# Vigilans/GomokuAI

Measured on AMD Instinct MI355X. Metric: board-evals/s, higher is better.
Workload: dtype int32; 1 GPU; batched AC-automaton position eval (K1), 65536 random-opening boards per GPU, 15x15, inputs resident in HBM; boards_per_gpu=65536, parallelism=boards sharded by rank, no collective, launch=hipGraph replay of the K steps

## Files before the change

### gomokuai_amd/csrc/capi.hip

```cpp
#include <algorithm>
#include <mutex>
#include <cstring>
#include <string>
#include <vector>

#include "capi_common.h"

namespace gmk {

static thread_local char g_error[512] = "";

void set_error(const char* fmt, ...) {
    va_list ap;
    va_start(ap, fmt);
    vsnprintf(g_error, sizeof g_error, fmt, ap);
    va_end(ap);
}

DeviceState& device_state() {
    static DeviceState s;
    return s;
}

}

using gmk::device_state;
using gmk::production_automaton;

extern "C" const char* gmk_last_error(void) { return gmk::g_error; }

namespace gmk {
namespace {
struct PoolBlock { void* p; size_t bytes; bool used; unsigned long long freed_at; };
unsigned long long g_pool_clock = 0;
std::mutex g_pool_mutex;
std::vector<PoolBlock> g_pool;
constexpr size_t kPoolMinBytes = size_t(16) << 20, kPoolCapBytes = size_t(224) << 30;
bool g_pool_poison = false;
size_t pool_idle_cap(size_t idle) {
    size_t free_bytes = 0, total = 0;
    if (hipMemGetInfo(&free_bytes, &total) != hipSuccess) { (void)hipGetLastError(); return kPoolCapBytes; }
    return std::min(kPoolCapBytes, (free_bytes + idle) / 4 * 3);
}
size_t pool_idle_bytes() { size_t t = 0; for (const PoolBlock& b : g_pool) if (!b.used) t += b.bytes; return t; }
void pool_drop_idle(size_t keep) {
    while (pool_idle_bytes() > keep) {
        size_t at = g_pool.size();
        for (size_t i = 0; i < g_pool.size(); ++i) if (!g_pool[i].used && (at == g_pool.size() || g_pool[i].freed_at < g_pool[at].freed_at)) at = i;
        if (at == g_pool.size()) return;
        (void)hipFree(g_pool[at].p);
        g_pool.erase(g_pool.begin() + static_cast<long>(at));
    }
}
}
// ... 90 lines not shown
    gmk::device_pool_release();
    (void)hipFree(st.d_trans);
    (void)hipFree(st.d_records);
    st = gmk::DeviceState{};
    return GMK_OK;
}

extern "C" int gmk_device_info(int* cu_count, size_t* hbm_bytes, char* name, int name_cap) {
    gmk::DeviceState& st = device_state();
    if (!st.ready) { gmk::set_error("gmk_init has not succeeded"); return GMK_ERR_STATE; }
    hipDeviceProp_t prop;
    GMK_HIP_CHECK(hipGetDeviceProperties(&prop, st.device));
    if (cu_count) *cu_count = prop.multiProcessorCount;
    if (hbm_bytes) *hbm_bytes = prop.totalGlobalMem;
    if (name && name_cap > 0) {
        std::strncpy(name, prop.name[0] ? prop.name : prop.gcnArchName, static_cast<size_t>(name_cap) - 1);
        name[name_cap - 1] = 0;
    }
    return GMK_OK;
}

extern "C" int gmk_tables_info(gmk_table_info* info) {
    if (!info) return GMK_ERR_ARG;
    const gmk::PatternAutomaton& a = production_automaton();
    const gmk::DeviceTables& t = a.device();
    info->n_patterns = t.n_patterns;
    info->n_states = t.n_states;
    info->dat_size = static_cast<int32_t>(a.base().size());
    info->max_emissions = t.max_emissions;
    info->trans_words = static_cast<int32_t>(t.trans.size());
    info->emit_words = static_cast<int32_t>(t.emit_lists.size());
    for (int i = 0; i < 5; ++i) info->invariants[i] = a.invariants()[i];
    return GMK_OK;
}

extern "C" int gmk_tables_pattern(int i, char str[8], int* favour, int* type, int* score) {
    const auto& pats = production_automaton().patterns();
    if (i < 0 || i >= static_cast<int>(pats.size())) return GMK_ERR_ARG;
    if (str) { std::memset(str, 0, 8); std::memcpy(str, pats[i].rich.data(), pats[i].rich.size()); }
    if (favour) *favour = pats[i].favour;
    if (type) *type = pats[i].type;
    if (score) *score = pats[i].score;
    return GMK_OK;
}

extern "C" int gmk_tables_copy(uint32_t* trans, uint16_t* emit_lists, uint32_t* pattern_info) {
    const gmk::DeviceTables& t = production_automaton().device();
    if (trans) std::memcpy(trans, t.trans.data(), t.trans.size() * sizeof(uint32_t));
    if (emit_lists) std::memcpy(emit_lists, t.emit_lists.data(), t.emit_lists.size() * sizeof(uint16_t));
    if (pattern_info) std::memcpy(pattern_info, t.pattern_info.data(), t.pattern_info.size() * sizeof(uint32_t));
    return GMK_OK;
}

extern "C" int gmk_tables_copy_dat(int32_t* base, int32_t* check, int32_t* fail) {
    const gmk::PatternAutomaton& a = production_automaton();
    const size_t bytes = a.base().size() * sizeof(int32_t);
    if (base) std::memcpy(base, a.base().data(), bytes);
    if (check) std::memcpy(check, a.check().data(), bytes);
    if (fail) std::memcpy(fail, a.fail().data(), bytes);
    return GMK_OK;
}

extern "C" int gmk_tables_scan(const uint8_t* codes, int n, int32_t* patterns, int32_t* offsets, int cap) {
    if (!codes || n < 0) return GMK_ERR_ARG;
    for (int i = 0; i < n; ++i) if (codes[i] < 1 || codes[i] > 4) return GMK_ERR_ARG;
    const auto stream = production_automaton().scan(codes, n);
    int m = 0;
    for (const auto& pr : stream) {
        if (m < cap) { if (patterns) patterns[m] = pr.first; if (offsets) offsets[m] = pr.second; }
        ++m;
    }
    return m;
}
```

### gomokuai_amd/csrc/eval_kernel.hip

```cpp
#include <algorithm>
#include <cstdlib>
#include <vector>

#include "capi_common.h"

namespace {

constexpr int kBoardsPerBlock = 16;
constexpr int kGroupBoards = 16;
constexpr int kThreads = 64 * kBoardsPerBlock;
constexpr int kCells = 225;
constexpr int kQueueCap = 448;
constexpr int kMaxBlocksPerCu = 1;
constexpr int kBurstEvery = 12;
static_assert(kBurstEvery >= 1 && kBurstEvery <= kGroupBoards, "every burst of a run needs a board of the run to go with");
[[maybe_unused]] constexpr int kTimelineSlots = 8;

constexpr int kScoreWords = 4 * kCells;
constexpr int kCntWords = 3 * kCells + 1;
constexpr int kZeroWords = kScoreWords + kCntWords;
constexpr int kLineWords = 96;
constexpr int kColBase = 20, kDiagBase = 36, kAntiBase = 65;
#ifndef GMK_K1_TOTALS_COPIES
#define GMK_K1_TOTALS_COPIES 8
#endif
constexpr int kTotalsCopies = GMK_K1_TOTALS_COPIES;
constexpr int kMiscWords = 48;
constexpr int kBoardWords = kZeroWords + kLineWords + kQueueCap + kMiscWords;
static_assert(kZeroWords % 4 == 0 && kBoardWords % 4 == 0, "16-byte alignment of the per-board blocks");
constexpr int kStaticTableWords = 128 + kLineWords + 512 + 1560 + 4;

constexpr int kLaneRecordVecs = 2;
constexpr int kScanSteps = 19;

__device__ __forceinline__ int dir_stride(int dir) { return (0x0E100F01u >> (8 * dir)) & 0xFFu; }

__device__ __forceinline__ uint64_t line_symbols(uint32_t line_word, int len) {
    return 2ull | (static_cast<uint64_t>(line_word) << 2) | (0xAull << (2 * len + 2));
}

__device__ __forceinline__ const __attribute__((address_space(3))) uint32_t* lds_word(uint32_t byte_address) {
    return reinterpret_cast<const __attribute__((address_space(3))) uint32_t*>(static_cast<uintptr_t>(byte_address));
}

__device__ __forceinline__ __attribute__((address_space(3))) uint32_t* lds_word_rw(uint32_t byte_address) {
    return reinterpret_cast<__attribute__((address_space(3))) uint32_t*>(static_cast<uintptr_t>(byte_address));
}

__device__ __forceinline__ uint32_t dfa_address(uint32_t table_word, uint32_t four) {
    uint32_t addr;
    asm("v_bfi_b32 %0, %1, %2, %3" : "=v"(addr) : "s"(0x3FF3u), "v"(table_word), "v"(four));
    return addr;
}

__device__ __forceinline__ uint32_t mul24(uint32_t a, uint32_t b) {
    uint32_t r;
    asm("v_mul_u32_u24 %0, %1, %2" : "=v"(r) : "v"(a), "s"(b));
    return r;
}

__device__ __forceinline__ void store_saddr(uint32_t byte_offset, int32_t value, unsigned long long base) {
    asm volatile("global_store_dword %0, %1, %2" : : "v"(byte_offset), "v"(value), "s"(base) : "memory");
}

template <int kImm, bool kNt>
__device__ __forceinline__ void store_saddr_imm(uint32_t byte_offset, int32_t value, unsigned long long base) {
    static_assert(kImm >= 0 && kImm < 4096, "the immediate offset of a global store has 13 bits, signed");
    if (kNt) asm volatile("global_store_dword %0, %1, %2 offset:%3 nt" : : "v"(byte_offset), "v"(value), "s"(base), "n"(kImm) : "memory");
    else asm volatile("global_store_dword %0, %1, %2 offset:%3" : : "v"(byte_offset), "v"(value), "s"(base), "n"(kImm) : "memory");
}

__device__ __forceinline__ void wave_phase_fence() {
    __builtin_amdgcn_fence(__ATOMIC_RELEASE, "wavefront");
    __builtin_amdgcn_wave_barrier();
    __builtin_amdgcn_fence(__ATOMIC_ACQUIRE, "wavefront");
}

__device__ __forceinline__ void deposit_match(uint32_t w0, uint32_t w1, int cell_at, int dir, int back_step,
                                              uint32_t* s_scores, uint32_t* s_cnt, uint32_t* s_misc, uint32_t* totals ) {
    const int type = w0 & 15, fav = (w0 >> 4) & 1;
    if (type == 8) { atomicOr(&s_misc[1], fav ? 1u : 2u); return; }
    atomicAdd(&totals[type], fav ? 0x10000u : 1u);
    const int endcell = cell_at + static_cast<int>((w0 >> 27) & 1u) * back_step;
    const uint32_t score = dir >= 2 ? (w1 >> 16) : (w1 & 0xFFFFu);
    unsigned long long* pair = reinterpret_cast<unsigned long long*>(s_scores) + fav;
    const uint32_t lo_opp = fav ? score : 0u, hi_opp = fav ? 0u : score;
    const uint32_t tslot = 5u - static_cast<uint32_t>(type);
    const bool feeds = tslot < 3u;
    uint32_t* cnt = s_cnt + (feeds ? tslot : 0u) * kCells;
    const uint32_t one = 1u << (4 * (fav * 4 + dir));
    const int n_dep = (w0 >> 8) & 7;
#pragma unroll
    for (int d = 0; d < 4; ++d) {
        if (d >= n_dep) break;
        const uint32_t f = (w0 >> (11 + 4 * d)) & 15u;
        const int c = endcell + static_cast<int>(f & 7u) * back_step;
        const bool both = (f & 8u) != 0u;
        atomicAdd(&pair[2 * c], (static_cast<unsigned long long>(both ? score : hi_opp) << 32) | (both ? score : lo_opp));
        if (both && feeds) atomicAdd(&cnt[c], one);
    }
}

__device__ __forceinline__ int counter_match(uint32_t w0, int k, int want) {
    const int type = w0 & 15, len = (w0 >> 5) & 7;
    const int back = k - static_cast<int>((w0 >> 27) & 1u) - 6;
    if (!w0 || type != want || back < 0 || back >= len) return -1;
    const int n_dep = (w0 >> 8) & 7;
    bool on_q = false;
#pragma unroll
    for (int d = 0; d < 4; ++d) {
        const uint32_t f = (w0 >> (11 + 4 * d)) & 15u;
        on_q |= d < n_dep && f == (8u | static_cast<uint32_t>(back));
    }
    return on_q ? back : -1;
}

__device__ __forceinline__ void add_counter_cells(uint32_t w0, int back, int q, int stride, uint32_t* opp) {
    const int n_dep = (w0 >> 8) & 7, endcell = q + back * stride;
#pragma unroll
    for (int d = 0; d < 4; ++d) {
        const uint32_t f = (w0 >> (11 + 4 * d)) & 15u;
        if (d < n_dep && static_cast<int>(f & 7u) != back) atomicAdd(&opp[4 * (endcell - static_cast<int>(f & 7u) * stride)], 600u);
    }
}

[[maybe_unused]] constexpr int kDensTiles = 7;
__host__ __device__ constexpr int dens_kt_lo(int m) { return (((32 * m) / 15 - 3) < 0 ? 0 : (32 * m) / 15 - 3) / 2; }
__host__ __device__ constexpr int dens_kt_hi(int m) { return (((32 * m + 31) / 15 + 3) > 14 ? 14 : (32 * m + 31) / 15 + 3) / 2; }
constexpr int kWtabDy = 13, kWtabEntryWords = 4, kWtabKindWords = kWtabDy * 15 * kWtabEntryWords, kWtabWords = 2 * kWtabKindWords;
__host__ __device__ constexpr int block_weight(int dy, int dx) {
    constexpr int w[4][7] = {{1, 3, 4, 0, 4, 3, 1}, {0, 3, 5, 4, 5, 3, 0}, {0, 4, 3, 3, 3, 4, 0}, {2, 0, 0, 1, 0, 0, 2}};
    return w[dy < 0 ? -dy : dy][dx + 3];
}

typedef int v4i __attribute__((ext_vector_type(4)));
typedef int v16i __attribute__((ext_vector_type(16)));

template <bool kFull, int KIND, int M>
__device__ __forceinline__ void density_tile_pass(const uint32_t (&own_rows)[8], int n_live, int lane,
                                                  const v4i* __restrict__ s_wtab, const uint4* __restrict__ s_occ, int32_t* __restrict__ group_out,
                                                  unsigned long long& board_base , const uint2* __restrict__ s_lut, int plane_stride) {
    constexpr int lo = dens_kt_lo(M), hi = dens_kt_hi(M), nk = hi - lo + 1;
    const int n = lane & 31, h = lane >> 5;
    const uint4 occ_lo = s_occ[4 * M + 2 * h], occ_hi = s_occ[4 * M + 2 * h + 1];
    const uint32_t occ[8] = {occ_lo.x, occ_lo.y, occ_lo.z, occ_lo.w, occ_hi.x, occ_hi.y, occ_hi.z, occ_hi.w};
    const int cell = 32 * M + n, yo = (cell * 0x8889) >> 19, xo = cell - 15 * yo;
    const v4i* w = s_wtab + KIND * (kWtabKindWords / kWtabEntryWords) + (2 * lo + h - yo + 6) * 15 + xo;
    v16i acc = {0, 0, 0, 0, 0, 0, 0, 0, 0, 0, 0, 0, 0, 0, 0, 0};
#pragma unroll
    for (int k = 0; k < nk; ++k) {
        const uint32_t r = (own_rows[lo + k] >> (16 * h)) & 0x7FFFu;
        const uint2 b0 = s_lut[r & 255u], b1 = s_lut[r >> 8];
// ... 595 lines not shown
        for (int k = 0; k < 2; ++k) {
            const uint32_t job = jobs[lane * 2 + k], dir = (job >> 5) & 3u, first = (job >> 12) & 255u;
            consts[lane][2 + k] = dir == 2u ? 2u * (first % 15u) : dir == 3u ? 2u * (first / 15u) : 0u;
        }
    }
    for (int i = 0; i < 128; ++i) jobs_out[i] = jobs[i];
    for (int i = 0; i < kLineWords; ++i) pads_out[i] = ~init[i] & 0xAAAAAAAAu;
    for (int lane = 0; lane < 64; ++lane) {
        uint32_t* r = records_out + 8 * lane;
        r[0] = jobs[lane * 2]; r[1] = jobs[lane * 2 + 1];
        r[2] = init[lane]; r[3] = init[std::min(64 + lane, kLineWords - 1)];
        for (int k = 0; k < 4; ++k) r[4 + k] = consts[lane][k];
    }
    if (steps != kScanSteps) { gmk::set_error("lane jobs: %d scan steps, the kernel is built for %d", steps, kScanSteps); return GMK_ERR_STATE; }
    return GMK_OK;
}

int density_weights(int8_t* t ) {
    for (int kind = 0; kind < 2; ++kind)
        for (int dy = -3; dy <= 3; ++dy)
            for (int xo = 0; xo < 15; ++xo)
                for (int j = 0; j < 15; ++j) {
                    if (std::abs(j - xo) > 3) continue;
                    const int w = block_weight(dy, j - xo);
                    t[((static_cast<size_t>(kind) * kWtabDy + dy + 6) * 15 + xo) * 16 + j] = static_cast<int8_t>(kind == 0 ? (w != 0) : w);
                }
    for (int cell = 0; cell < 224; ++cell)
        for (int kt = dens_kt_lo(cell / 32); kt <= dens_kt_hi(cell / 32); ++kt)
            for (int h = 0; h < 2; ++h) {
                const int dy = 2 * kt + h - cell / 15;
                if (dy < -6 || dy > 6) { gmk::set_error("density weight table: dy %d of cell %d out of range", dy, cell); return GMK_ERR_STATE; }
            }
    for (int cell = 0; cell < 224; ++cell)
        for (int dy = -3; dy <= 3; ++dy) {
            const int y = cell / 15 + dy, m = cell / 32;
            if (y < 0 || y > 14) continue;
            if (y / 2 < dens_kt_lo(m) || y / 2 > dens_kt_hi(m)) { gmk::set_error("density weight table: row %d of cell %d is not covered", y, cell); return GMK_ERR_STATE; }
        }
    return GMK_OK;
}

int build_stage_image(const gmk::DeviceState& st, uint4** d_out, int* stage_vecs) {
    const size_t trans_words = static_cast<size_t>(st.n_states) * 4, record_words = static_cast<size_t>(st.n_records) * 4;
    std::vector<uint32_t> rest(kStaticTableWords + 64 * 4 * kLaneRecordVecs, 0u);
    uint32_t* jobs = rest.data(), *pads = jobs + 128, *lut = pads + kLineWords, *wtab = lut + 512, *handout = wtab + kWtabWords, *records = handout + 4;
    int rc = lane_tables(jobs, pads, records);
    if (rc != GMK_OK) return rc;
    for (uint32_t b = 0; b < 256; ++b) { lut[2 * b] = ((b & 15u) * 0x204081u) & 0x01010101u; lut[2 * b + 1] = ((b >> 4) * 0x204081u) & 0x01010101u; }
    rc = density_weights(reinterpret_cast<int8_t*>(wtab));
    if (rc != GMK_OK) return rc;
    handout[0] = 2u * kBoardsPerBlock;
    const size_t staged_words = trans_words + record_words + kStaticTableWords;
    if (staged_words % 4 != 0) { gmk::set_error("K1 tables: %zu staged words are not whole 16-byte pieces", staged_words); return GMK_ERR_STATE; }
    uint32_t* d = nullptr;
    GMK_HIP_CHECK(hipMalloc(&d, (trans_words + record_words + rest.size()) * sizeof(uint32_t)));
    GMK_HIP_CHECK(hipMemcpy(d, st.d_trans, trans_words * sizeof(uint32_t), hipMemcpyDeviceToDevice));
    GMK_HIP_CHECK(hipMemcpy(d + trans_words, st.d_records, record_words * sizeof(uint32_t), hipMemcpyDeviceToDevice));
    GMK_HIP_CHECK(hipMemcpy(d + trans_words + record_words, rest.data(), rest.size() * sizeof(uint32_t), hipMemcpyHostToDevice));
    *d_out = reinterpret_cast<uint4*>(d);
    *stage_vecs = static_cast<int>(staged_words / 4);
    return GMK_OK;
}

struct Launch { int grid, n_groups, groups_each, groups_extra; size_t lds; };

Launch plan_launch(int n, const gmk::DeviceState& st) {
    Launch l;
    l.n_groups = (n + kGroupBoards - 1) / kGroupBoards;
    l.grid = std::max(1, std::min(l.n_groups, st.cu_count * kMaxBlocksPerCu));
    l.groups_each = l.n_groups / l.grid;
    l.groups_extra = l.n_groups % l.grid;
    l.lds = static_cast<size_t>(kBoardsPerBlock * kBoardWords + st.n_states * 4 + st.n_records * 4 + kStaticTableWords) * 4;
    return l;
}

bool g_jobs_uploaded = false;
uint4* g_stage = nullptr;
int g_stage_vecs = 0;
}

extern "C" int gmk_eval_batch(const uint16_t* d_planes, int n, int32_t* d_scores, int32_t* d_density,
                              uint32_t* d_totals, int32_t* d_status, void* stream) {
    gmk::DeviceState& st = gmk::device_state();
    if (!st.ready) { gmk::set_error("gmk_init has not succeeded (no CPU fallback)"); return GMK_ERR_STATE; }
    if (n < 0 || (n > 0 && !d_planes)) { gmk::set_error("gmk_eval_batch: bad arguments"); return GMK_ERR_ARG; }
    if (n == 0) return GMK_OK;
    if (!g_jobs_uploaded) {
        const int rc = build_stage_image(st, &g_stage, &g_stage_vecs);
        if (rc != GMK_OK) return rc;
        GMK_HIP_CHECK(hipFuncSetAttribute(reinterpret_cast<const void*>(eval_positions_kernel), hipFuncAttributeMaxDynamicSharedMemorySize, 160 * 1024));
        g_jobs_uploaded = true;
    }
    const Launch l = plan_launch(n, st);
    if (l.lds > 160u * 1024u) { gmk::set_error("gmk_eval_batch: tables do not fit in LDS (%zu bytes)", l.lds); return GMK_ERR_CAPACITY; }
    static const int phase_mask = gmk::profile_env("GMK_EVAL_PHASE_MASK") ? std::atoi(gmk::profile_env("GMK_EVAL_PHASE_MASK")) : 0x7F;
    unsigned long long* d_prof = nullptr;
    static const bool stamps = gmk::profile_env("GMK_EVAL_PROFILE") != nullptr;
    if (stamps) {
        GMK_HIP_CHECK(hipMalloc(&d_prof, 16 * sizeof(unsigned long long)));
        GMK_HIP_CHECK(hipMemset(d_prof, 0, 16 * sizeof(unsigned long long)));
    }
    static const char* const timeline_path = gmk::profile_env("GMK_EVAL_TIMELINE");
    unsigned long long* d_timeline = nullptr;
    const size_t timeline_words = static_cast<size_t>(l.grid) * kBoardsPerBlock * kTimelineSlots;
    hipEvent_t tl_from = nullptr, tl_to = nullptr;
    if (timeline_path) {
        GMK_HIP_CHECK(hipMalloc(&d_timeline, timeline_words * sizeof(unsigned long long)));
        GMK_HIP_CHECK(hipMemset(d_timeline, 0, timeline_words * sizeof(unsigned long long)));
        GMK_HIP_CHECK(hipEventCreate(&tl_from));
        GMK_HIP_CHECK(hipEventCreate(&tl_to));
// ... 75 lines not shown
```

### gomokuai_amd/csrc/pattern_tables.cpp

```cpp
#include "pattern_tables.h"

#include <algorithm>
#include <deque>
#include <map>
#include <numeric>
#include <stdexcept>

namespace gmk {

namespace {

constexpr int kMaxLen = 7;
constexpr int kSymbols = 4;

std::vector<PatternRec> production_protos() {
    struct P { const char* s; int type; int score; };
    static const P table[] = {
        {"+xxxxx", Five, 9999},      {"-_oooo_", LiveFour, 9000},   {"-xoooo_", DeadFour, 2500},
        {"-o_ooo", DeadFour, 3000},  {"-oo_oo", DeadFour, 2600},    {"-~_ooo_~", LiveThree, 3000},
        {"-x^ooo_~", LiveThree, 2900}, {"-~o_oo~", LiveThree, 2800}, {"-~o~oo_~", DeadThree, 1400},
        {"-~oo~o_~", DeadThree, 1200}, {"-x_o~oo~", DeadThree, 1300}, {"-x_oo~o~", DeadThree, 1100},
        {"-xooo__~", DeadThree, 510}, {"-xoo_o_~", DeadThree, 520},  {"-xoo__o~", DeadThree, 520},
        {"-xo_oo_~", DeadThree, 530}, {"-xo__oo", DeadThree, 530},   {"-xooo__x", DeadThree, 500},
        {"-xoo_o_x", DeadThree, 500}, {"-xoo__ox", DeadThree, 500},  {"-xo_oo_x", DeadThree, 500},
// ... 300 lines not shown
        dev_.dev_prefix4[idx] = static_cast<uint16_t>(row);
    }

    {
        const int n = dev_.n_states;
        std::vector<std::vector<uint32_t>> frontier(1), next_frontier;
        frontier[0].resize(static_cast<size_t>(n));
        for (int i = 0; i < n; ++i) frontier[0][static_cast<size_t>(i)] = static_cast<uint32_t>(i);
        int length = 0;
        while (!frontier.empty()) {
            if (++length > 12) throw std::runtime_error("pattern automaton: does not forget its start state within 12 symbols");
            next_frontier.clear();
            std::vector<char> seen(static_cast<size_t>(n));
            for (const std::vector<uint32_t>& set : frontier)
                for (uint32_t sym = 0; sym < 4; ++sym) {
                    std::fill(seen.begin(), seen.end(), 0);
                    std::vector<uint32_t> image;
                    for (uint32_t st : set) {
                        const uint32_t to = dev_.trans[st * 4 + sym] & 1023u;
                        if (!seen[to]) { seen[to] = 1; image.push_back(to); }
                    }
                    if (image.size() > 1) next_frontier.push_back(std::move(image));
                }
            frontier.swap(next_frontier);
        }
        dev_.sync_symbols = length;
        if (length > 7) throw std::runtime_error("pattern automaton: needs more than 7 symbols to forget its start state");
    }
}

std::vector<std::pair<int, int>> PatternAutomaton::scan(const uint8_t* codes, int n) const {
    std::vector<std::pair<int, int>> out;
    uint32_t state = 0;
    for (int k = 0; k < n; ++k) {
        const uint32_t w = dev_.trans[state * 4 + (codes[k] - 1)];
        state = w & 1023u;
        const uint32_t li = w >> 10;
        if (li) {
            const int cnt = dev_.emit_lists[li];
            for (int e = 0; e < cnt; ++e) {
                const uint16_t v = dev_.emit_lists[li + 1 + e];
                out.emplace_back(v & 0x7fff, k - (v >> 15));
            }
        }
    }
    return out;
}

const PatternAutomaton& production_automaton() {
    static const PatternAutomaton a;
    return a;
}

}
```

### gomokuai_amd/csrc/pattern_tables.h

```cpp
#pragma once
#include <cstdint>
#if defined(__HIP__)
#include <hip/hip_runtime.h>
#endif
#include <string>
#include <vector>

namespace gmk {

enum PatternType : int { DeadOne, LiveOne, DeadTwo, LiveTwo, DeadThree, LiveThree, DeadFour, LiveFour, Five, NumPatternTypes };

struct PatternRec {
    std::string rich;
    int favour;
    int type;
    int score;
};

inline int symbol_code(char ch) {
    switch (ch) { case 'x': return 1; case 'o': return 2; case '?': return 3;
                  case '-': case '_': case '^': case '~': return 4; default: return 0; }
}

struct Emission { uint16_t pattern; uint8_t back; };
// ... 5 lines not shown
#endif
GMK_TABLE_FN uint32_t dev_trans_row(uint32_t tw) { return tw & 0x3FFFu; }
GMK_TABLE_FN uint32_t dev_trans_kinds(uint32_t tw) { return (tw >> 14) & 7u; }
GMK_TABLE_FN uint32_t dev_trans_record(uint32_t tw) { return tw >> 17; }
constexpr int kPrefixWords = 128;

struct DeviceTables {
    std::vector<uint32_t> trans;
    std::vector<uint16_t> emit_lists;
    std::vector<uint32_t> pattern_info;
    std::vector<uint32_t> dev_trans;
    std::vector<uint32_t> dev_records;
    int n_records = 0;
    std::vector<uint16_t> dev_prefix4;
    int sync_symbols = 0;
    int n_states = 0;
    int n_patterns = 0;
    int max_emissions = 0;
};

class PatternAutomaton {
public:
    PatternAutomaton();
    explicit PatternAutomaton(const std::vector<PatternRec>& protos);

    const std::vector<PatternRec>& patterns() const { return patterns_; }
    const std::vector<int>& base() const { return base_; }
    const std::vector<int>& check() const { return check_; }
    const std::vector<int>& fail() const { return fail_; }
    const std::vector<int>& invariants() const { return invariants_; }
    const DeviceTables& device() const { return dev_; }

    std::vector<std::pair<int, int>> scan(const uint8_t* codes, int n) const;

private:
    void augment();
    void sort_patterns();
    void build_trie();
    void build_double_array();
    void build_fail_links();
    void flatten();
    bool terminal(int s) const { return check_[base_[s]] == s; }
    int pattern_of(int s) const { return -base_[base_[s]]; }

    struct TrieNode { int code, depth, first, last; };
    std::vector<TrieNode> trie_;
    std::vector<PatternRec> patterns_;
    std::vector<int> base_, check_, fail_, invariants_;
    DeviceTables dev_;
};

const PatternAutomaton& production_automaton();

}
```

### gomokuai_amd/lib.py

```python
import ctypes as C
import os

import numpy as np

_HERE = os.path.dirname(os.path.abspath(__file__))
_SO = os.path.join(_HERE, "libgomoku_hip.so")
if os.environ.get("GMK_HIP_LIB") == "prof":
    _SO = os.path.join(_HERE, "libgomoku_hip_prof.so")
elif os.environ.get("GMK_HIP_LIB", "").endswith(".so"):
    _SO = os.environ["GMK_HIP_LIB"]

N = 225


class GmkError(RuntimeError):
    pass


class TableInfo(C.Structure):
    _fields_ = [("n_patterns", C.c_int32), ("n_states", C.c_int32), ("dat_size", C.c_int32),
                ("max_emissions", C.c_int32), ("trans_words", C.c_int32), ("emit_words", C.c_int32),
                ("invariants", C.c_int32 * 5)]


_lib = None

OPT_NOISE_SAMPLER, OPT_LOCKSTEP = 1, 2
NOISE_SAMPLERS = {"std": 0, "counter": 1}

EXPORTS = [
    "gmk_init", "gmk_shutdown", "gmk_pool_release", "gmk_pool_poison", "gmk_last_error", "gmk_device_info",
    "gmk_tables_info", "gmk_tables_pattern", "gmk_tables_copy", "gmk_tables_copy_dat", "gmk_tables_scan",
    "gmk_synth_boards", "gmk_moves_to_planes",
    "gmk_eval_batch", "gmk_eval_batch_host", "gmk_eval_launch_info",
    "gmk_mcts_create", "gmk_mcts_destroy", "gmk_mcts_set_roots", "gmk_mcts_set_game_ids", "gmk_mcts_run", "gmk_mcts_root_stats",
    "gmk_mcts_alg_bytes", "gmk_mcts_launch_info", "gmk_visits_to_pi", "gmk_mcts_advance", "gmk_mcts_step", "gmk_mcts_step_host", "gmk_mcts_add_root_noise", "gmk_mcts_set_option", "gmk_mcts_reserve", "gmk_selfplay_run", "gmk_samples_from_records",
    "gmk_records_scan", "gmk_records_packed_bytes", "gmk_records_pack", "gmk_records_unpack", "gmk_samples_from_packed",
    "gmk_evalstate_create", "gmk_evalstate_destroy", "gmk_evalstate_reset", "gmk_evalstate_update", "gmk_evalstate_update_host", "gmk_evalstate_read",
    "gmk_az_create", "gmk_az_destroy", "gmk_az_set_roots", "gmk_az_select", "gmk_az_expand", "gmk_az_select_host", "gmk_az_expand_host", "gmk_az_read_node_host", "gmk_az_read_children_host", "gmk_az_set_leaf_host", "gmk_az_rollout_host", "gmk_az_expand_stages_host", "gmk_az_write_stats_host", "gmk_az_step", "gmk_az_advance", "gmk_az_set_slots", "gmk_az_live_games", "gmk_az_set_game_ids", "gmk_az_add_root_noise", "gmk_az_set_option", "gmk_az_root_stats",
    "gmk_trad_create", "gmk_trad_destroy", "gmk_trad_reset_evaluators", "gmk_trad_set_game_ids", "gmk_trad_set_positions", "gmk_trad_run", "gmk_trad_step", "gmk_trad_add_root_noise", "gmk_trad_set_option", "gmk_trad_reserve", "gmk_trad_root_stats", "gmk_trad_read_evaluators", "gmk_trad_run_poolrave", "gmk_trad_run_rave", "gmk_trad_root_amaf", "gmk_trad_selfplay_run", "gmk_pvnet_create", "gmk_pvnet_destroy", "gmk_pvnet_forward", "gmk_pvnet_set_dense", "gmk_pvnet_evaluate",
    "gmk_pattern_policy", "gmk_pattern_policy_host", "gmk_pattern_play",
    "gmk_replay_create", "gmk_replay_destroy", "gmk_replay_reset", "gmk_replay_append", "gmk_replay_append_packed", "gmk_replay_size",
    "gmk_replay_sample", "gmk_replay_draw_host",
]


def _torch_first():
    try:
        import torch
    except ImportError:
        return
    if torch.cuda.is_available():
        torch.cuda.init()


def load():
    global _lib
    if _lib is not None:
        return _lib
    _torch_first()
    if not os.path.exists(_SO):
        raise GmkError("libgomoku_hip.so is missing: run `python -m gomokuai_amd.build` "
                       "(there is no CPU fallback for the compute path)")
    L = C.CDLL(_SO)
    vp = C.c_void_p
    L.gmk_last_error.restype = C.c_char_p
    L.gmk_init.argtypes = [C.c_int]
    L.gmk_device_info.argtypes = [C.POINTER(C.c_int), C.POINTER(C.c_size_t), C.c_char_p, C.c_int]
    L.gmk_tables_info.argtypes = [C.POINTER(TableInfo)]
    L.gmk_tables_pattern.argtypes = [C.c_int, C.c_char_p, C.POINTER(C.c_int), C.POINTER(C.c_int), C.POINTER(C.c_int)]
    L.gmk_tables_copy.argtypes = [vp, vp, vp]
    L.gmk_tables_copy_dat.argtypes = [vp, vp, vp]
    L.gmk_tables_scan.argtypes = [vp, C.c_int, vp, vp, C.c_int]
    L.gmk_synth_boards.argtypes = [C.c_uint64, C.c_uint32, C.c_int, C.c_int, vp, C.c_int, vp, vp]
    L.gmk_moves_to_planes.argtypes = [vp, C.c_int, vp, C.c_int, vp]
    L.gmk_eval_batch.argtypes = [vp, C.c_int, vp, vp, vp, vp, vp]
    L.gmk_eval_batch_host.argtypes = [vp, C.c_int, vp, vp, vp, vp]
    L.gmk_eval_launch_info.argtypes = [C.c_int, C.POINTER(C.c_int), C.POINTER(C.c_int), C.POINTER(C.c_int)]
    L.gmk_mcts_create.argtypes = [C.c_int, C.c_int, C.c_double, C.c_int, C.c_uint64, C.POINTER(vp)]
    L.gmk_mcts_destroy.argtypes = [vp]
    L.gmk_mcts_set_roots.argtypes = [vp, vp, vp, C.c_uint32]
    L.gmk_mcts_set_game_ids.argtypes = [vp, vp]
    L.gmk_trad_set_game_ids.argtypes = [vp, vp]
    L.gmk_az_set_game_ids.argtypes = [vp, vp]
    L.gmk_mcts_run.argtypes = [vp, C.c_int, vp]
    L.gmk_mcts_root_stats.argtypes = [vp, vp, vp, vp, vp, vp]
    L.gmk_mcts_alg_bytes.argtypes = [vp, C.POINTER(C.c_uint64)]
    L.gmk_mcts_launch_info.argtypes = [vp, C.POINTER(C.c_int), C.POINTER(C.c_int), C.POINTER(C.c_int)]
    L.gmk_visits_to_pi.argtypes = [vp, C.c_int, vp]
    L.gmk_mcts_advance.argtypes = [vp, vp, vp, vp, vp, vp, C.c_int, vp]
    L.gmk_mcts_step.argtypes = [vp, vp, vp, vp, vp, vp, vp, C.c_int, vp]
    L.gmk_mcts_step_host.argtypes = [vp, vp, C.c_int]
    L.gmk_selfplay_run.argtypes = [vp, C.c_int, C.c_uint32, C.c_int, C.c_int, C.c_float, C.c_float, vp, C.c_int, vp, vp, vp, vp, vp, C.POINTER(C.c_int32), vp]
    L.gmk_mcts_add_root_noise.argtypes = [vp, C.c_float, C.c_float, vp]
    L.gmk_mcts_set_option.argtypes = [vp, C.c_int, C.c_int]
    L.gmk_mcts_reserve.argtypes = [vp, C.c_int]
    L.gmk_trad_reserve.argtypes = [vp, C.c_int]
    L.gmk_evalstate_create.argtypes = [C.c_int, C.POINTER(vp)]
    L.gmk_evalstate_destroy.argtypes = [vp]
    L.gmk_evalstate_reset.argtypes = [vp]
    L.gmk_evalstate_update.argtypes = [vp, vp, C.c_int, vp]
    L.gmk_evalstate_update_host.argtypes = [vp, vp, C.c_int]
    L.gmk_evalstate_read.argtypes = [vp, vp, vp, vp, vp, vp, vp]
    L.gmk_az_create.argtypes = [C.c_int, C.c_int, C.c_double, C.POINTER(vp)]
    L.gmk_az_destroy.argtypes = [vp]
    L.gmk_az_set_roots.argtypes = [vp, vp, vp]
    L.gmk_az_select.argtypes = [vp, vp, vp]
    L.gmk_az_expand.argtypes = [vp, vp, vp, vp]
    L.gmk_az_select_host.argtypes = [vp, vp, vp]
    L.gmk_az_step.argtypes = [vp, vp]
    L.gmk_az_live_games.argtypes = [vp, C.POINTER(C.c_int32)]
    L.gmk_az_set_slots.argtypes = [vp, C.c_int, vp, C.c_int, vp]
    L.gmk_az_advance.argtypes = [vp, vp, vp, vp, vp, C.c_int, C.POINTER(C.c_int32), vp]
    L.gmk_az_add_root_noise.argtypes = [vp, C.c_float, C.c_float, C.c_uint64, C.c_uint32]
    L.gmk_az_set_option.argtypes = [vp, C.c_int, C.c_int]
    L.gmk_az_expand_host.argtypes = [vp, vp, vp]
    L.gmk_az_root_stats.argtypes = [vp] * 8
    L.gmk_trad_create.argtypes = [C.c_int, C.c_int, C.POINTER(vp)]
    L.gmk_trad_destroy.argtypes = [vp]
    L.gmk_trad_reset_evaluators.argtypes = [vp]
    L.gmk_trad_set_positions.argtypes = [vp, vp, vp]
    L.gmk_trad_run.argtypes = [vp, C.c_int, C.c_double, vp]
    L.gmk_trad_step.argtypes = [vp, vp]
    L.gmk_trad_add_root_noise.argtypes = [vp, C.c_float, C.c_float, C.c_uint64, C.c_uint32]
    L.gmk_trad_set_option.argtypes = [vp, C.c_int, C.c_int]
    L.gmk_trad_root_stats.argtypes = [vp] * 10
# ... 36 lines not shown


def init(device=0):
    _check(load().gmk_init(device))


def pool_poison(on=True):
    _check(load().gmk_pool_poison(1 if on else 0))


def release_pool():
    _check(load().gmk_pool_release())


def device_info():
    cu = C.c_int()
    mem = C.c_size_t()
    name = C.create_string_buffer(256)
    _check(load().gmk_device_info(C.byref(cu), C.byref(mem), name, 256))
    return {"cu_count": cu.value, "hbm_bytes": mem.value, "name": name.value.decode()}


def tables_info():
    info = TableInfo()
    _check(load().gmk_tables_info(C.byref(info)))
    return info


def tables_pattern(i):
    s = C.create_string_buffer(8)
    fav, typ, score = C.c_int(), C.c_int(), C.c_int()
    _check(load().gmk_tables_pattern(i, s, C.byref(fav), C.byref(typ), C.byref(score)))
    return s.value.decode(), fav.value, typ.value, score.value


def tables_copy():
    info = tables_info()
    trans = np.zeros(info.trans_words, dtype=np.uint32)
    emit = np.zeros(info.emit_words, dtype=np.uint16)
    pinfo = np.zeros(info.n_patterns * 2, dtype=np.uint32)
    _check(load().gmk_tables_copy(trans.ctypes.data, emit.ctypes.data, pinfo.ctypes.data))
    return trans, emit, pinfo


def tables_copy_dat():
    info = tables_info()
    base = np.zeros(info.dat_size, dtype=np.int32)
    check = np.zeros(info.dat_size, dtype=np.int32)
    fail = np.zeros(info.dat_size, dtype=np.int32)
    _check(load().gmk_tables_copy_dat(base.ctypes.data, check.ctypes.data, fail.ctypes.data))
    return base, check, fail


def tables_scan(codes):
    codes = np.ascontiguousarray(codes, dtype=np.uint8)
    pats = np.zeros(512, dtype=np.int32)
    offs = np.zeros(512, dtype=np.int32)
    m = _check(load().gmk_tables_scan(codes.ctypes.data, len(codes), pats.ctypes.data, offs.ctypes.data, 512))
    return list(zip(pats[:m].tolist(), offs[:m].tolist()))


DEFAULT_SEED = 0x9E3779B97F4A7C15


def synth_boards(n, kind=0, seed=DEFAULT_SEED, first_board=0, stride=64):
    moves = np.zeros((n, stride), dtype=np.uint8)
    lens = np.zeros(n, dtype=np.int32)
    planes = np.zeros((n, 2, 16), dtype=np.uint16)
    _check(load().gmk_synth_boards(seed, first_board, n, kind, moves.ctypes.data, stride, lens.ctypes.data, planes.ctypes.data))
    return moves, lens, planes


def moves_to_planes(moves, lens):
    moves = np.ascontiguousarray(moves, dtype=np.uint8)
    lens = np.ascontiguousarray(lens, dtype=np.int32)
    n, stride = moves.shape
    planes = np.zeros((n, 2, 16), dtype=np.uint16)
    _check(load().gmk_moves_to_planes(moves.ctypes.data, stride, lens.ctypes.data, n, planes.ctypes.data))
    return planes


def eval_batch_host(planes):
    init()
    planes = np.ascontiguousarray(planes, dtype=np.uint16)
    n = planes.shape[0]
    scores = np.zeros((n, 4, N), dtype=np.int32)
    density = np.zeros((n, 2, 2, N), dtype=np.int32)
    totals = np.zeros((n, 11), dtype=np.uint32)
    status = np.zeros(n, dtype=np.int32)
    _check(load().gmk_eval_batch_host(planes.ctypes.data, n, scores.ctypes.data, density.ctypes.data,
                                      totals.ctypes.data, status.ctypes.data))
    return scores, density, totals, status


def eval_batch(d_planes, n, d_scores=None, d_density=None, d_totals=None, d_status=None, stream=None):
    _check(load().gmk_eval_batch(d_planes, n, d_scores, d_density, d_totals, d_status, stream))


def eval_launch_info(n):
    g, b, l = C.c_int(), C.c_int(), C.c_int()
    _check(load().gmk_eval_launch_info(n, C.byref(g), C.byref(b), C.byref(l)))
    return {"grid": g.value, "block": b.value, "lds_bytes": l.value}


class BatchedMCTS:

# ... 475 lines not shown
```

### include/gomoku_hip.h

```cpp
#ifndef GOMOKU_HIP_H_
#define GOMOKU_HIP_H_
#include <stddef.h>
#include <stdint.h>

#ifdef __cplusplus
extern "C" {
#endif

typedef enum {
    GMK_OK = 0,
    GMK_ERR_NO_DEVICE = -1,
    GMK_ERR_HIP = -2,
    GMK_ERR_ARG = -3,
    GMK_ERR_STATE = -4,
    GMK_ERR_CAPACITY = -5
} gmk_status;

enum { GMK_BOARD_CELLS = 225, GMK_PLANE_WORDS = 16, GMK_TOTALS = 11 };

int gmk_init(int device);
int gmk_shutdown(void);
int gmk_pool_release(void);
int gmk_pool_poison(int on);
const char *gmk_last_error(void);
int gmk_device_info(int *cu_count, size_t *hbm_bytes, char *name, int name_cap);

typedef struct {
    int32_t n_patterns;
    int32_t n_states;
    int32_t dat_size;
    int32_t max_emissions;
    int32_t trans_words;
    int32_t emit_words;
    int32_t invariants[5];
} gmk_table_info;
int gmk_tables_info(gmk_table_info *info);
int gmk_tables_pattern(int i, char str[8], int *favour, int *type, int *score);
int gmk_tables_copy(uint32_t *trans, uint16_t *emit_lists, uint32_t *pattern_info);
int gmk_tables_copy_dat(int32_t *base, int32_t *check, int32_t *fail);
int gmk_tables_scan(const uint8_t *codes, int n, int32_t *patterns, int32_t *offsets, int cap);

int gmk_synth_boards(uint64_t seed, uint32_t first_board, int n, int kind,
                     uint8_t *h_moves, int stride, int32_t *h_lens, uint16_t *h_planes);
int gmk_moves_to_planes(const uint8_t *h_moves, int stride, const int32_t *h_lens, int n, uint16_t *h_planes);

int gmk_eval_batch(const uint16_t *d_planes, int n,
                   int32_t *d_scores, int32_t *d_density, uint32_t *d_totals, int32_t *d_status,
                   void *stream);
int gmk_eval_batch_host(const uint16_t *h_planes, int n,
                        int32_t *h_scores, int32_t *h_density, uint32_t *h_totals, int32_t *h_status);
int gmk_eval_launch_info(int n, int *grid, int *block, int *lds_bytes);

typedef struct gmk_evalstate gmk_evalstate;
int gmk_evalstate_create(int n_games, gmk_evalstate **out);
int gmk_evalstate_destroy(gmk_evalstate *e);
int gmk_evalstate_reset(gmk_evalstate *e);
int gmk_evalstate_update(gmk_evalstate *e, const int16_t *d_moves, int moves_per_game, void *stream);
int gmk_evalstate_update_host(gmk_evalstate *e, const int16_t *h_moves, int moves_per_game);
int gmk_evalstate_read(gmk_evalstate *e, int32_t *h_scores, int32_t *h_density, uint32_t *h_pattern_dist, uint32_t *h_compound_dist,
                       int32_t *h_meta, uint8_t *h_record);

typedef struct gmk_mcts gmk_mcts;
int gmk_mcts_create(int n_games, int node_capacity, double c_puct, int c_rollouts, uint64_t seed, gmk_mcts **out);
int gmk_mcts_destroy(gmk_mcts *m);
int gmk_mcts_set_roots(gmk_mcts *m, const uint16_t *h_planes, const int16_t *h_last_move, uint32_t first_game_id);
int gmk_mcts_set_game_ids(gmk_mcts *m, const uint32_t *h_ids);
int gmk_mcts_run(gmk_mcts *m, int playouts, void *stream);
int gmk_mcts_advance(gmk_mcts *m, uint8_t *d_moves, uint16_t *d_visits, int32_t *d_lens, int8_t *d_winner,
                     int32_t *d_unfinished, int reuse_subtree, void *stream);
int gmk_selfplay_run(gmk_mcts *m, int n_total, uint32_t first_game_id, int playouts, int reuse_subtree, float noise_alpha, float noise_epsilon,
                     const uint8_t *h_open_moves, int open_stride, const int32_t *h_open_lens,
                     uint8_t *d_moves, uint16_t *d_visits, int32_t *d_lens, int8_t *d_winner, int32_t *h_steps, void *stream);
int gmk_mcts_step(gmk_mcts* m, const int16_t* d_forced_moves, uint8_t* d_moves, uint16_t* d_visits, int32_t* d_lens,
                  int8_t* d_winner, int32_t* d_unfinished, int reuse_subtree, void* stream);
int gmk_mcts_step_host(gmk_mcts* m, const int16_t* h_moves, int reuse_subtree);
int gmk_mcts_add_root_noise(gmk_mcts *m, float alpha, float epsilon, void *stream);
enum { GMK_OPT_NOISE_SAMPLER = 1, GMK_OPT_LOCKSTEP = 2 };
enum { GMK_NOISE_SAMPLER_STD = 0, GMK_NOISE_SAMPLER_COUNTER = 1 };
int gmk_mcts_set_option(gmk_mcts *m, int option, int value);
int gmk_mcts_reserve(gmk_mcts *m, int two_arenas);
int gmk_mcts_root_stats(gmk_mcts *m, uint32_t *h_visits, float *h_root_value, uint32_t *h_root_visits,
                        uint32_t *h_nodes, int32_t *h_status);
int gmk_mcts_alg_bytes(gmk_mcts *m, uint64_t *bytes);
int gmk_mcts_launch_info(gmk_mcts *m, int *grid, int *block, int *lds_bytes);
int gmk_visits_to_pi(const uint32_t *visits, int stones, float *pi);

int gmk_samples_from_records(const uint8_t *d_moves, const int32_t *d_lens, const uint16_t *d_visits, const int8_t *d_winner,
                             const int32_t *d_sample_game, const int32_t *d_sample_move, int n_samples, int augment,
                             uint8_t *d_states, float *d_values, float *d_pi, void *stream);

enum { GMK_WIRE_BAD_LENGTH = 1, GMK_WIRE_BAD_SIZE = 2 };
int gmk_records_scan(const int32_t *d_lens, int n, int64_t *d_offsets, void *stream);
int gmk_records_packed_bytes(const int64_t *d_offsets, int n, int has_visits, uint64_t *h_bytes, void *stream);
// ... 95 lines not shown
```

Baseline: 579.9 million board-evals/s.

## Presort K1 match deposits into both/opponent groups and use direct LDS addressing

Records for the K1 kernel are rewritten on the host so each match lists its '_' (both-sides) deposits before its '^' (opponent-only) deposits, with the count of the first group stored in spare bits 28..30. The kernel then runs two separate unrolled loops: one does a 64-bit add of the score into both halves plus the threat-count increment, the other does a single 32-bit add into the opponent slot. This removes per-deposit select logic and the 64-bit add that carried a zero half. LDS addresses are computed with v_mad_i32_i24 and raw address-space-3 pointers. Host-side validation throws if a record exceeds the unrolled bounds.

```diff
diff --git a/gomokuai_amd/csrc/capi.hip b/gomokuai_amd/csrc/capi.hip
--- a/gomokuai_amd/csrc/capi.hip
+++ b/gomokuai_amd/csrc/capi.hip
@@ -1,5 +1,6 @@
 #include <algorithm>
 #include <mutex>
+#include <stdexcept>
 #include <cstring>
 #include <string>
 #include <vector>
@@ -196,6 +197,17 @@
     return GMK_OK;
 }
 
+extern "C" int gmk_tables_records(uint32_t* shared, uint32_t* k1) {
+    const gmk::DeviceTables& t = production_automaton().device();
+    try {
+        const std::vector<uint32_t>& own = gmk::production_k1_records();
+        if (own.size() != t.dev_records.size()) { gmk::set_error("K1 records: %zu words, the shared records have %zu", own.size(), t.dev_records.size()); return GMK_ERR_STATE; }
+        if (shared) std::memcpy(shared, t.dev_records.data(), t.dev_records.size() * sizeof(uint32_t));
+        if (k1) std::memcpy(k1, own.data(), own.size() * sizeof(uint32_t));
+    } catch (const std::exception& e) { gmk::set_error("%s", e.what()); return GMK_ERR_STATE; }
+    return t.n_records;
+}
+
 extern "C" int gmk_tables_copy_dat(int32_t* base, int32_t* check, int32_t* fail) {
     const gmk::PatternAutomaton& a = production_automaton();
     const size_t bytes = a.base().size() * sizeof(int32_t);
diff --git a/gomokuai_amd/csrc/eval_kernel.hip b/gomokuai_amd/csrc/eval_kernel.hip
--- a/gomokuai_amd/csrc/eval_kernel.hip
+++ b/gomokuai_amd/csrc/eval_kernel.hip
@@ -1,5 +1,6 @@
 #include <algorithm>
 #include <cstdlib>
+#include <stdexcept>
 #include <vector>
 
 #include "capi_common.h"
@@ -59,6 +60,17 @@
     return r;
 }
 
+__device__ __forceinline__ uint32_t mad24(int a, int b, uint32_t c) {
+    uint32_t r;
+    asm("v_mad_i32_i24 %0, %1, %2, %3" : "=v"(r) : "v"(a), "v"(b), "v"(c));
+    return r;
+}
+
+template <int kOffset>
+__device__ __forceinline__ __attribute__((address_space(3))) char* lds_byte_rw(uint32_t byte_address) {
+    return reinterpret_cast<__attribute__((address_space(3))) char*>(static_cast<uintptr_t>(byte_address)) + kOffset;
+}
+
 __device__ __forceinline__ void store_saddr(uint32_t byte_offset, int32_t value, unsigned long long base) {
     asm volatile("global_store_dword %0, %1, %2" : : "v"(byte_offset), "v"(value), "s"(base) : "memory");
 }
@@ -83,21 +95,30 @@
     atomicAdd(&totals[type], fav ? 0x10000u : 1u);
     const int endcell = cell_at + static_cast<int>((w0 >> 27) & 1u) * back_step;
     const uint32_t score = dir >= 2 ? (w1 >> 16) : (w1 & 0xFFFFu);
-    unsigned long long* pair = reinterpret_cast<unsigned long long*>(s_scores) + fav;
-    const uint32_t lo_opp = fav ? score : 0u, hi_opp = fav ? 0u : score;
+    const int step16 = back_step * 16, step4 = back_step * 4;
+    const uint32_t wave_at = static_cast<uint32_t>(reinterpret_cast<uintptr_t>(s_scores)) - 4u * kStaticTableWords;
+    const uint32_t pair_at = wave_at + static_cast<uint32_t>(endcell * 16 + fav * 8);
+    const uint32_t opp_at = pair_at + 4u * static_cast<uint32_t>(fav ^ 1);
+    const unsigned long long both_value = (static_cast<unsigned long long>(score) << 32) | score;
     const uint32_t tslot = 5u - static_cast<uint32_t>(type);
     const bool feeds = tslot < 3u;
-    uint32_t* cnt = s_cnt + (feeds ? tslot : 0u) * kCells;
+    const uint32_t cnt_at = wave_at + static_cast<uint32_t>(static_cast<int>(feeds ? tslot : 0u) * (kCells * 4) + endcell * 4);
     const uint32_t one = 1u << (4 * (fav * 4 + dir));
-    const int n_dep = (w0 >> 8) & 7;
-#pragma unroll
-    for (int d = 0; d < 4; ++d) {
-        if (d >= n_dep) break;
-        const uint32_t f = (w0 >> (11 + 4 * d)) & 15u;
-        const int c = endcell + static_cast<int>(f & 7u) * back_step;
-        const bool both = (f & 8u) != 0u;
-        atomicAdd(&pair[2 * c], (static_cast<unsigned long long>(both ? score : hi_opp) << 32) | (both ? score : lo_opp));
-        if (both && feeds) atomicAdd(&cnt[c], one);
+    const int n_dep = (w0 >> 8) & 7, n_both = (w0 >> 28) & 7;
+#pragma unroll
+    for (int d = 0; d < gmk::kK1MaxBoth; ++d) {
+        if (d >= n_both) break;
+        const int piece = static_cast<int>(__builtin_amdgcn_ubfe(w0, 11 + 4 * d, 3));
+        atomicAdd((unsigned long long*)lds_byte_rw<4 * kStaticTableWords>(mad24(piece, step16, pair_at)), both_value);
+        if (feeds) atomicAdd((uint32_t*)lds_byte_rw<4 * (kStaticTableWords + kScoreWords)>(mad24(piece, step4, cnt_at)), one);
+    }
+    const uint32_t rest = w0 >> (11 + 4 * n_both);
+    const int n_opp = n_dep - n_both;
+#pragma unroll
+    for (int d = 0; d < gmk::kK1MaxOpp; ++d) {
+        if (d >= n_opp) break;
+        const int piece = static_cast<int>(__builtin_amdgcn_ubfe(rest, 4 * d, 3));
+        atomicAdd((uint32_t*)lds_byte_rw<4 * kStaticTableWords>(mad24(piece, step16, opp_at)), score);
     }
 }
 
@@ -799,10 +820,13 @@
     handout[0] = 2u * kBoardsPerBlock;
     const size_t staged_words = trans_words + record_words + kStaticTableWords;
     if (staged_words % 4 != 0) { gmk::set_error("K1 tables: %zu staged words are not whole 16-byte pieces", staged_words); return GMK_ERR_STATE; }
+    const std::vector<uint32_t>* own_records = nullptr;
+    try { own_records = &gmk::production_k1_records(); } catch (const std::exception& e) { gmk::set_error("%s", e.what()); return GMK_ERR_STATE; }
+    if (own_records->size() != record_words) { gmk::set_error("K1 records: %zu words, the device state has %zu", own_records->size(), record_words); return GMK_ERR_STATE; }
     uint32_t* d = nullptr;
     GMK_HIP_CHECK(hipMalloc(&d, (trans_words + record_words + rest.size()) * sizeof(uint32_t)));
     GMK_HIP_CHECK(hipMemcpy(d, st.d_trans, trans_words * sizeof(uint32_t), hipMemcpyDeviceToDevice));
-    GMK_HIP_CHECK(hipMemcpy(d + trans_words, st.d_records, record_words * sizeof(uint32_t), hipMemcpyDeviceToDevice));
+    GMK_HIP_CHECK(hipMemcpy(d + trans_words, own_records->data(), record_words * sizeof(uint32_t), hipMemcpyHostToDevice));
     GMK_HIP_CHECK(hipMemcpy(d + trans_words + record_words, rest.data(), rest.size() * sizeof(uint32_t), hipMemcpyHostToDevice));
     *d_out = reinterpret_cast<uint4*>(d);
     *stage_vecs = static_cast<int>(staged_words / 4);
diff --git a/gomokuai_amd/csrc/pattern_tables.cpp b/gomokuai_amd/csrc/pattern_tables.cpp
--- a/gomokuai_amd/csrc/pattern_tables.cpp
+++ b/gomokuai_amd/csrc/pattern_tables.cpp
@@ -376,4 +376,37 @@
     return a;
 }
 
-}
+std::vector<uint32_t> k1_records(const std::vector<uint32_t>& dev_records) {
+    std::vector<uint32_t> out(dev_records);
+    for (size_t m = 0; m + 1 < out.size(); m += 2) {
+        const uint32_t w0 = dev_records[m];
+        if (w0 >> 28) throw std::runtime_error("K1 records: bits 28..31 of a record's first word are taken");
+        const int n_dep = static_cast<int>((w0 >> 8) & 7u);
+        if (n_dep > 4) throw std::runtime_error("K1 records: a match has more than four deposits");
+        uint32_t both[4], opp[4];
+        int n_both = 0, n_opp = 0;
+        for (int d = 0; d < n_dep; ++d) {
+            const uint32_t f = (w0 >> (11 + 4 * d)) & 15u;
+            if (f & 8u) both[n_both++] = f; else opp[n_opp++] = f;
+        }
+        if (n_both > kK1MaxBoth || n_opp > kK1MaxOpp) throw std::runtime_error("K1 records: a match has more '_' or '^' deposits than the kernel's loops are unrolled for");
+        uint32_t w = (w0 & ~(0xFFFFu << 11)) | (static_cast<uint32_t>(n_both) << 28);
+        for (int d = 0; d < n_dep; ++d) w |= (d < n_both ? both[d] : opp[d - n_both]) << (11 + 4 * d);
+        int seen[16] = {};
+        for (int d = 0; d < 4; ++d) {
+            if (d < n_dep) { ++seen[(w0 >> (11 + 4 * d)) & 15u]; --seen[(w >> (11 + 4 * d)) & 15u]; }
+            else if ((w >> (11 + 4 * d)) & 15u) throw std::runtime_error("K1 records: a field behind a match's last deposit is not zero");
+        }
+        for (int f = 0; f < 16; ++f) if (seen[f]) throw std::runtime_error("K1 records: a match's deposits differ from its source record's");
+        if ((w ^ w0) & ~((0xFFFFu << 11) | (7u << 28))) throw std::runtime_error("K1 records: a bit outside the deposit fields changed");
+        out[m] = w;
+    }
+    return out;
+}
+
+const std::vector<uint32_t>& production_k1_records() {
+    static const std::vector<uint32_t> r = k1_records(production_automaton().device().dev_records);
+    return r;
+}
+
+}
diff --git a/gomokuai_amd/csrc/pattern_tables.h b/gomokuai_amd/csrc/pattern_tables.h
--- a/gomokuai_amd/csrc/pattern_tables.h
+++ b/gomokuai_amd/csrc/pattern_tables.h
@@ -81,4 +81,9 @@
 
 const PatternAutomaton& production_automaton();
 
+constexpr int kK1MaxBoth = 4;
+constexpr int kK1MaxOpp = 2;
+std::vector<uint32_t> k1_records(const std::vector<uint32_t>& dev_records);
+const std::vector<uint32_t>& production_k1_records();
+
 }
diff --git a/gomokuai_amd/lib.py b/gomokuai_amd/lib.py
--- a/gomokuai_amd/lib.py
+++ b/gomokuai_amd/lib.py
@@ -30,7 +30,7 @@
 
 EXPORTS = [
     "gmk_init", "gmk_shutdown", "gmk_pool_release", "gmk_pool_poison", "gmk_last_error", "gmk_device_info",
-    "gmk_tables_info", "gmk_tables_pattern", "gmk_tables_copy", "gmk_tables_copy_dat", "gmk_tables_scan",
+    "gmk_tables_info", "gmk_tables_pattern", "gmk_tables_copy", "gmk_tables_copy_dat", "gmk_tables_scan", "gmk_tables_records",
     "gmk_synth_boards", "gmk_moves_to_planes",
     "gmk_eval_batch", "gmk_eval_batch_host", "gmk_eval_launch_info",
     "gmk_mcts_create", "gmk_mcts_destroy", "gmk_mcts_set_roots", "gmk_mcts_set_game_ids", "gmk_mcts_run", "gmk_mcts_root_stats",
@@ -72,6 +72,7 @@
     L.gmk_tables_copy.argtypes = [vp, vp, vp]
     L.gmk_tables_copy_dat.argtypes = [vp, vp, vp]
     L.gmk_tables_scan.argtypes = [vp, C.c_int, vp, vp, C.c_int]
+    L.gmk_tables_records.argtypes = [vp, vp]
     L.gmk_synth_boards.argtypes = [C.c_uint64, C.c_uint32, C.c_int, C.c_int, vp, C.c_int, vp, vp]
     L.gmk_moves_to_planes.argtypes = [vp, C.c_int, vp, C.c_int, vp]
     L.gmk_eval_batch.argtypes = [vp, C.c_int, vp, vp, vp, vp, vp]
@@ -214,6 +215,14 @@
     return base, check, fail
 
 
+def tables_records():
+    n = _check(load().gmk_tables_records(None, None))
+    shared = np.zeros((n, 4), dtype=np.uint32)
+    k1 = np.zeros((n, 4), dtype=np.uint32)
+    _check(load().gmk_tables_records(shared.ctypes.data, k1.ctypes.data))
+    return shared, k1
+
+
 def tables_scan(codes):
     codes = np.ascontiguousarray(codes, dtype=np.uint8)
     pats = np.zeros(512, dtype=np.int32)
diff --git a/include/gomoku_hip.h b/include/gomoku_hip.h
--- a/include/gomoku_hip.h
+++ b/include/gomoku_hip.h
@@ -39,6 +39,7 @@
 int gmk_tables_copy(uint32_t *trans, uint16_t *emit_lists, uint32_t *pattern_info);
 int gmk_tables_copy_dat(int32_t *base, int32_t *check, int32_t *fail);
 int gmk_tables_scan(const uint8_t *codes, int n, int32_t *patterns, int32_t *offsets, int cap);
+int gmk_tables_records(uint32_t *shared, uint32_t *k1);
 
 int gmk_synth_boards(uint64_t seed, uint32_t first_board, int n, int kind,
                      uint8_t *h_moves, int stride, int32_t *h_lens, uint16_t *h_planes);
```

After: 581.4 million board-evals/s, median of 6. About the same (+0.3%).
